# chto/linna

Measured on AMD Instinct MI355X. Metric: emulator log-likelihood evals/sec, higher is better.
Workload: dtype f32; 1 GPU; 33-D Gaussian, 4x512 MLP emulator (33->512x4->33), nwalkers=4096 batched log-likelihood per GPU (BASELINE configs[1]); nwalkers_per_gpu=4096, launch=direct launches, parallelism=walkers sharded, 1 rank(s), no data-path collective

## Files before the change

### linna_amd/csrc/net_stream.hip

```cpp
#include "common.h"
#include <stdlib.h>
#include <type_traits>
#include <vector>
#include <cstring>
#include <algorithm>
#include <atomic>
#include <memory>
#include <mutex>
#include <string>
#include <unordered_map>

namespace linna {

typedef __bf16 bf16x8 __attribute__((ext_vector_type(8)));
typedef short s16x4 __attribute__((ext_vector_type(4)));

constexpr int NS_ROWS = 16;
constexpr int NS_NW = 8;
constexpr int NS_NT = 4;
constexpr int NS_MAXSEG = 20;
constexpr int NS_MAXRUN = 40;
constexpr unsigned NS_STEP_B = NS_NT * 1024;
constexpr int NS_LDS_BYTES = 160 * 1024;
#ifndef NS_R
// ... 412 lines not shown
            in_ext[i] = (NS_NW / ncg) * s.kslice;
            q.bias_pad = 64 * ncg; q.ncg = ncg;
        } else {
            s.type = NS_WIDE; s.steps = ksteps; s.passes = passes;
            in_ext[i] = KS * ksteps;
            q.bias_pad = 512 * passes; q.ncg = 1;
        }
        q.Wa = L.Wa; q.lda = L.lda; q.Ka = L.Ka; q.Kapad = L.Kapad; q.Wb = L.Wb; q.ldb = L.ldb; q.Kb = L.Kb; q.alpha = L.alpha;
        q.b = L.b; q.bscale = L.bscale; q.N = L.N; q.type = s.type; q.steps = s.steps; q.passes = s.passes; q.bias_off = bias_off;
        q.transA = L.transA; q.transB = L.transB; q.rscale = L.rscale; q.rshift = L.rshift; q.b2 = L.b2; q.b2scale = L.b2scale;
        q.kc = side ? kc : 1; q.side_off = 0;
        s.x0_col = L.x0_col; s.x0_n = L.x0_col ? ceil16(L.Kb) : 0;
        if (L.transA && !dx_prog) {
            if (zero_off < 0) { zero_off = bias_off; zero_pad = 0; }
            s.bias_off = q.bias_off = zero_off;
            const int grow = std::max(0, q.bias_pad - zero_pad);
            zero_pad += grow; q.bias_pad = grow;
        }
        bias_off += q.bias_pad;
        if (dn && dn->tri > 0 && s.type == NS_WIDE && dn->factored && L.Wa == dn->S && passes == 2 && ksteps > 32 && !train) {
            if (dn->tri == 2 && (L.N + 63) / 64 == 16 && ksteps > 60) s.zext = -1;
            else { s.kslice = 512; s.zext = ksteps - 32; }
        }
        q.koff2 = s.type == NS_WIDE ? (s.zext < 0 ? -1 : s.kslice) : 0;
        if (!side) G += ns_seg_steps(s);
        p.seg.push_back(s); p.pack.push_back(q);
    }
    if (want_grad) {
        int slot = 0;
        for (int i = 0; i < nfwd - 1; ++i) {
            if (p.seg[i].type != NS_WIDE) { want_grad = false; break; }
            p.seg[i].mask_store = 1 + slot;
            slot += p.seg[i].passes;
        }
        for (size_t j = nfwd; j < lins.size() && want_grad; ++j) {
            const int of = lins[j].mask_apply_of;
            if (of < 0) continue;
            if (p.seg[j].type != NS_WIDE || p.seg[j].passes != p.seg[of].passes) { want_grad = false; break; }
            p.seg[j].mask_apply = p.seg[of].mask_store;
        }
        if (want_grad) p.mask_slots = slot;
        else {
            for (size_t j = lins.size(); j-- > (size_t)nfwd;) { G -= ns_seg_steps(p.seg[j]); bias_off -= p.pack[j].bias_pad; }
            p.seg.resize(nfwd); p.pack.resize(nfwd); lins.resize(nfwd); in_ext.resize(nfwd);
            for (int i = 0; i < nfwd; ++i) p.seg[i].mask_store = 0;
        }
    }
    int Gf = 0;
    for (int i = 0; i < nfwd; ++i) if (p.seg[i].type != NS_SIDE) Gf += ns_seg_steps(p.seg[i]);

    p.kpad0 = in_ext[0];
    int def = p.kpad0, writer = -1;
    int maxext = 64;
    for (size_t i = 0; i < p.seg.size(); ++i) {
        NsSeg& s = p.seg[i];
        if (in_ext[i] > def) {
            if (writer == -1) p.kpad0 = def = in_ext[i];
            else if (writer >= 0) { NsSeg& w = p.seg[writer]; w.zext = in_ext[i] - w.dst_col; def = in_ext[i]; }
            else return p;
        }
        maxext = std::max(maxext, in_ext[i]);
        if (s.type == NS_WIDE) {
            if (s.dst_col != 0) return p;
            def = 512 * s.passes; writer = -2;
            maxext = std::max(maxext, def);
        } else {
            if (s.dst_col > def) return p;
            if (s.dst_col == 0) def = s.zext;
            else def = std::max(def, s.dst_col + s.zext);
            writer = (int)i;
        }
    }
    for (const NsSeg& s : p.seg) if (s.type != NS_WIDE) maxext = std::max(maxext, s.dst_col + s.zext);
    if (p.kpad0 > (dx_prog ? 1024 : bf ? 512 : 256)) return p;
    p.bf = bf; p.f32seg = f32seg;
    p.nout = lins[nfwd - 1].N;
    p.G = Gf; p.Gstride = G; p.nseg_f = nfwd; p.grad_ok = want_grad;
    for (size_t i = 0; i < lins.size(); ++i) { p.seg_op.push_back(lins[i].op); p.seg_hidden.push_back(lins[i].same_buf ? 1 : 0); }
    p.dxi_ok = fwd_dxi;
    p.train_ok = train;
    p.bias_total = bias_off;
    p.LD = std::max(((maxext + 63) & ~63) + 4, 516);
    if (bias_off > 3 * 64 * NS_NW * 4) return p;
    p.lds_bytes = (size_t)(2 * NS_ROWS * p.LD + ((bias_off + 3) & ~3)) * sizeof(float) + 128 + (p.x0_keep ? 4096 : 0);
#ifdef NS_STAMPS
    p.lds_bytes += NS_NW * 32 * 8;
#endif
    if (p.lds_bytes > (size_t)NS_LDS_BYTES) return p;
    p.lds_bytes_grad = p.lds_bytes + (size_t)p.mask_slots * 64 * NS_NW * sizeof(unsigned);
    if (p.grad_ok && p.lds_bytes_grad > (size_t)NS_LDS_BYTES) return p;
    int nrun = 0;
    for (const NsSeg& s : p.seg) nrun += s.passes;
    if (nrun > NS_MAXRUN) return p;
    p.packed_floats = (size_t)NS_NW * G * NS_NT * 256 + (size_t)((bias_off + 3) & ~3);
    for (size_t i = 0; i < p.seg.size(); ++i)
        if (p.seg[i].type == NS_SIDE) {
            p.seg[i].side_off = p.pack[i].side_off = (int)p.packed_floats;
            p.packed_floats += (size_t)NS_NW * p.seg[i].steps * NS_NT * 256;
            p.side_f4 += (size_t)NS_NW * p.seg[i].steps * NS_NT * 64;
        }
    p.ok = true;
    return p;
}

static std::atomic<int> g_forced_rows{-1};
static int ns_forced_rows_resolved() {
    int forced = g_forced_rows.load(std::memory_order_relaxed);
    if (forced < 0) {
        const char* const env = getenv("LINNA_NS_ROWS");
        const int v = env ? atoi(env) : 0;
        forced = (v == 4 || v == 8 || v == 16) ? v : 0;
        int expect = -1;
        g_forced_rows.compare_exchange_strong(expect, forced);
        forced = g_forced_rows.load(std::memory_order_relaxed);
    }
    return forced;
}
int net_stream_force_rows(int rows) {
    if (rows != 0 && rows != 4 && rows != 8 && rows != 16) return -1;
    (void)ns_forced_rows_resolved();
    return g_forced_rows.exchange(rows);
}
int net_stream_rows(int B) {
    const int forced = ns_forced_rows_resolved();
    if (forced) return forced;
    static int ncu = 0;
    if (!ncu) {
        int dev = 0; hipDeviceProp_t pr;
        ncu = (hipGetDevice(&dev) == hipSuccess && hipGetDeviceProperties(&pr, dev) == hipSuccess && pr.multiProcessorCount > 0)
                  ? pr.multiProcessorCount : 256;
    }
    return B <= 4 * ncu ? 4 : B <= 8 * ncu ? 8 : 16;
}

static bool ns_side(NsKind kind, int rows) {
    return rows == 16 && (kind == NS_SERVE || kind == NS_SERVE_DENSE || kind == NS_GRAD_INPUT);
}

static NsProgram ns_build_kind(NsKind kind, const linna_layer_t* layers, int nl, int in_size, const NsDense* dn, bool side) {
    NsProgram p;
    switch (kind) {
    case NS_SERVE: case NS_STORE:
        p = ns_build_one(layers, nl, in_size, NS_PROG_FWD, nullptr, side);
        if (!p.ok) p = ns_build_one(layers, nl, in_size, NS_PROG_FWD_NOGRAD, nullptr, side);
        break;
    case NS_SERVE_DENSE: case NS_TRAIN_FWD: p = ns_build_one(layers, nl, in_size, NS_PROG_FWD_DENSE, dn, side); break;
    case NS_SERVE_BF16: p = ns_build_one(layers, nl, in_size, NS_PROG_FWD_NOGRAD, dn, false, true); break;
    case NS_DX: p = ns_build_one(layers, nl, in_size, NS_PROG_DX); break;
    case NS_DX_INPUT: p = ns_build_one(layers, nl, in_size, NS_PROG_DX_INPUT); break;
    case NS_GRAD_INPUT: p = ns_build_one(layers, nl, in_size, NS_PROG_FWD_DXI, nullptr, side); break;
    case NS_TRAIN_STEP: p = ns_build_one(layers, nl, in_size, NS_PROG_TRAIN, dn); break;
    case NS_TRAIN_STEP_BF16: p = ns_build_one(layers, nl, in_size, NS_PROG_TRAIN, dn, false, true); break;
    }
    if (side && !(p.ok && (kind != NS_GRAD_INPUT || p.dxi_ok))) return ns_build_kind(kind, layers, nl, in_size, dn, false);
    return p;
}
typedef std::shared_ptr<const NsProgram> NsProgramRef;
static NsProgramRef ns_program(NsKind kind, const linna_layer_t* layers, int nl, int in_size, const NsDense* dn, int rows) {
    static std::mutex mu;
    static std::unordered_map<std::string, NsProgramRef> cache;
    const bool side = ns_side(kind, rows);
    std::string key;
    key.reserve((size_t)nl * sizeof(linna_layer_t) + 64);
    key.append(reinterpret_cast<const char*>(layers), (size_t)nl * sizeof(linna_layer_t));
    const int hdr[4] = {nl, in_size, (int)kind, side ? 1 : 0};
    key.append(reinterpret_cast<const char*>(hdr), sizeof(hdr));
// ... 586 lines not shown
```

### linna_amd/csrc/net_stream_body.inc

```
    constexpr int NT = NS_NT, NW = NS_NW;
    constexpr int RG = 32;
    constexpr bool SM = ROWS < 16;
    constexpr int RS = SM ? ROWS / 4 : 1;
    constexpr int NQ = SM ? RS : NT;
    constexpr int NACC = SM ? 4 * RS : NT;
#ifdef NS_BODY_SLICE_BF16
    static_assert(BF && !GRAD && STORE == 0 && MOVE == 2, "bf16: the slice evaluation");
#else
    static_assert(!BF || (!GRAD && STORE == 0 && MOVE != 2) || (GRAD && STORE == 3 && MOVE == 0 && ROWS == 4),
                  "bf16: serving, the fused stretch move and the merged training step (4-row engine)");
#endif
    constexpr bool BFT = BF && GRAD && STORE == 3;
    constexpr int AK = BF ? 2 : 1;
    constexpr bool K4 = !SM && !BF && (STORE == 0 || (GRAD && STORE == 2));
    constexpr bool TRB = GRAD && STORE == 3;
    constexpr bool DXE = STORE == 2 || TRB;
    constexpr bool G2 = GRAD && STORE == 2;
    constexpr bool LB = G2;
    constexpr bool LATE_REFILL = true;
    static_assert(ROWS == 16 || ROWS == 8 || ROWS == 4, "rows per workgroup");
    static_assert(R % 2 == 0, "the A double buffer alternates with the ring slot parity");
    extern __shared__ __attribute__((aligned(16))) float smem[];
    const int LD = a.LD, ABUF = ROWS * LD;
    constexpr bool KA = STORE == 3 || STORE == 1 || GRAD;
    const NsArgs* const ka = KA ? reinterpret_cast<const NsArgs*>((const void*)__builtin_amdgcn_kernarg_segment_ptr()) : &a;
    float* const act = smem;
    float* const lbias = smem + 2 * ABUF;
    unsigned* const lbits = reinterpret_cast<unsigned*>(smem + a.bits_off);
    const int nbw = a.nbw;
    const int tid = threadIdx.x, lane = tid & 63;
    const int wave = __builtin_amdgcn_readfirstlane(tid >> 6);
    const int li = lane & 15, kq = lane >> 4;
    const int row0 = blockIdx.x * ROWS;
    if (a.gate && a.gate[0] == 0) return;
    int mv_rows = a.B;
    if constexpr (MOVE == 2) {
        if (a.mv_C) {
            mv_rows = a.mv_step[0] * a.mv_step_off;
            if (row0 >= mv_rows) return;
        }
    }
    if constexpr ((STORE == 2 && !GRAD) || TRB) {
        if ((a.p_n > 0 || a.p_step) && blockIdx.x == gridDim.x - 1) {
            float* const part = smem;
            float acc0 = 0.f, acc1 = 0.f;
            for (int i = tid; i < a.p_n; i += 1024) acc0 += a.p_rows[i];
            for (int i = tid + 512; i < a.p_n; i += 1024) acc1 += a.p_rows[i];
#pragma unroll
            for (int o = 32; o >= 1; o >>= 1) { acc0 += __shfl_xor(acc0, o, 64); acc1 += __shfl_xor(acc1, o, 64); }
            if (lane == 0) { part[wave] = acc0; part[8 + wave] = acc1; }
            __syncthreads();
            if (tid == 0 && a.p_out) {
                float t = 0.f;
                for (int w = 0; w < 16; ++w) t += part[w];
                a.p_out[0] = t * a.p_scale;
            }
            if (tid == 64 && a.p_step) {
                const int t = ++a.p_step[0];
                a.p_hyper[2] = (float)(1.0 - pow((double)a.p_b1, (double)t));
                a.p_hyper[3] = (float)sqrt(1.0 - pow((double)a.p_b2, (double)t));
            }
            return;
        }
    }
#ifdef NS_STAMPS
    unsigned long long* const lstamp = reinterpret_cast<unsigned long long*>(lbias + ((a.bias_total + 3) & ~3) + 32 + (a.x0_keep ? 1024 : 0)) + wave * 32;
    int nstamp = 0;
#define NS_STAMP() do { const unsigned long long t_ = __builtin_readcyclecounter(); \
        if (lane == 0 && nstamp < 32) lstamp[nstamp] = t_; ++nstamp; } while (0)
#define NS_STAMPS_FLUSH() do { if (lane < 32) a.stamps[((size_t)blockIdx.x * NW + wave) * 32 + lane] = lane < nstamp ? lstamp[lane] : 0ull; } while (0)
#else
#define NS_STAMP() do {} while (0)
#define NS_STAMPS_FLUSH() do {} while (0)
#endif
    NS_STAMP();

    const int prt = tid / RG, pc0 = tid % RG;
    const bool prow = prt < ROWS;
    const int pr = SM ? min(prt, ROWS - 1) : prt;
    int grow = min(row0 + pr, a.B - 1);
    if constexpr (MOVE == 2) {
        if (a.mv_C) grow = a.mv_C[min(row0 + pr, mv_rows - 1)];
    }
    int zsrc = grow;
    float zden = 1.f;
    if constexpr (STORE == 3) {
        zsrc = a.t_rows ? a.t_rows[grow] : grow;
        zden = a.t_den[zsrc];
    }
    const int kpad0 = a.kpad0, nin = a.nin, nout = a.nout, nseg = a.nseg;
    const int nlast = (TRB ? a.nseg_f : nseg) - 2;
    constexpr int ZPRE = 2;
    float zr[ZPRE], za1[ZPRE], za2[ZPRE], zxm[ZPRE], zxs[ZPRE]; int zfl[ZPRE], zlg[ZPRE];
    const int* const lgp = a.lg ? a.lg : a.is_flat;
    int mv_wk = 0; float mv_factor = 0.f, mv_lnp_old = 0.f, mv_logu = 0.f;
    if constexpr (MOVE == 1) {
        mv_wk = a.mv_S[grow];
        const U4 rb = walker_bits(a.mv_seed, (uint32_t)mv_wk, (uint32_t)(a.mv_step[0] + a.mv_step_off), (uint32_t)a.mv_stream, 0u);
        const float t = (a.mv_a - 1.f) * u01(rb.x) + 1.f;
        const float zf = t * t / a.mv_a;
        const int j = (int)(((uint64_t)rb.y * (uint64_t)a.mv_nc) >> 32);
        const int wc = a.mv_C[j];
// ... 3 lines not shown
#pragma unroll
        for (int i = 0; i < ZPRE; ++i) {
            const int c = min(pc0 + i * RG, nin - 1);
            const float cr = a.mv_cc[(size_t)wc * a.mv_ldcc + c], sx = a.mv_coords[(size_t)mv_wk * a.mv_ldc + c];
            zr[i] = cr - (cr - sx) * zf;
        }
    }
    if constexpr (MOVE == 2) {
        const int k = grow % a.mv_nc;
        const int wk = a.mv_S[k];
        float wgt;
        if (a.sb.logp) {
            const SliceBegin& b = a.sb;
            const int jt = grow / a.mv_nc;
            const U4 rb = walker_bits(b.seed, (uint32_t)wk, (uint32_t)b.step[0], (uint32_t)b.half, 0u);
            const int ia = (int)(((uint64_t)rb.x * (uint64_t)b.nc) >> 32);
            int ib = (int)(((uint64_t)rb.y * (uint64_t)(b.nc - 1)) >> 32);
            ib += (ib >= ia);
            const int wa = b.C[ia], wb = b.C[ib];
            const float mu = b.mu[0];
            const float l = -u01(rb.w);
            wgt = jt < b.m ? l - (float)jt : l + 1.f + (float)(jt - b.m);
            const bool first = jt == 0 && prow && row0 + pr < a.B;
#pragma unroll
            for (int i = 0; i < ZPRE; ++i) {
                const int c = min(pc0 + i * RG, nin - 1);
                const float dir = mu * (b.cc[(size_t)wa * b.ldcc + c] - b.cc[(size_t)wb * b.ldcc + c]);
                zr[i] = a.mv_coords[(size_t)wk * a.mv_ldc + c] + wgt * dir;
                if (first && pc0 + i * RG < nin) b.DIR[(size_t)k * b.ldd + c] = dir;
            }
            if (first && pc0 == 0) {
                b.Z0[k] = b.logp[wk] + logf(u01(rb.z));
                b.L[k] = l; b.R[k] = l + 1.f;
                int J, K;
                slice_budget(b.seed, (uint32_t)wk, (uint32_t)b.step[0], (uint32_t)b.half, b.maxsteps, J, K);
                b.flags[3 * k] = J; b.flags[3 * k + 1] = K; b.flags[3 * k + 2] = 1;
            }
            if (blockIdx.x == 0 && tid == 0) {
                for (int i = 0; i < b.nslots; ++i) {
                    b.counters[4 + b.nslots + i] += b.counters[4 + i];
                    b.counters[4 + i] = 0;
                }
                b.counters[4 + 2 * b.nslots] += 1;
                if (b.zero_totals) { b.counters[0] = 0; b.counters[1] = 0; }
            }
        } else {
        if (a.sl_Zt) {
            const int ns_ = a.mv_nc, m = a.sl_m, jt = grow / ns_;
            const float z0 = a.sl_Z0[k];
            const float zend = a.sl_Zt[(size_t)min(pc0, 2 * m - 1) * ns_ + k];
            const unsigned long long bal = __ballot(pc0 < 2 * m && zend > z0);
            const unsigned bits = (unsigned)(bal >> (lane & 32));
            const unsigned lm = bits & ((1u << m) - 1u), rm = (bits >> m) & ((1u << m) - 1u);
            const int nl = min(__builtin_ctz(~lm), a.sl_flags[3 * k]), nr = min(__builtin_ctz(~rm), a.sl_flags[3 * k + 1]);
            float l = a.sl_L[k], r = a.sl_R[k];
            for (int j = 0; j < m; ++j) {
                if (j < nl) l -= 1.f;
                if (j < nr) r += 1.f;
            }
            const U4 tb = walker_bits(a.sl_seed, (uint32_t)wk, (uint32_t)a.sl_step[0], (uint32_t)a.sl_stream, (uint32_t)(pc0 + 1));
            const int myu = __float_as_int(u01(tb.x));
            wgt = 0.f;
            for (int jj = 0; jj < a.sl_nt; ++jj) {
                const int ulo = __builtin_amdgcn_readlane(myu, jj), uhi = __builtin_amdgcn_readlane(myu, 32 + jj);
                const float u = __int_as_float((lane & 32) ? uhi : ulo);
                const float w = l + u * (r - l);
                if (jj == jt) wgt = w;
                if (jj < jt) { if (w < 0.f) l = w; else r = w; }
            }
        } else {
            wgt = a.mv_cc[grow];
        }
#pragma unroll
        for (int i = 0; i < ZPRE; ++i) {
            const int c = min(pc0 + i * RG, nin - 1);
            zr[i] = a.mv_coords[(size_t)wk * a.mv_ldc + c] + wgt * a.Z[(size_t)k * a.ldz + c];
        }
        }
    }
#pragma unroll
    for (int i = 0; i < ZPRE; ++i) {
        const int c = min(pc0 + i * RG, nin - 1);
        if constexpr (MOVE == 0) zr[i] = a.Z[(size_t)(STORE == 3 ? zsrc : grow) * a.ldz + c];
        zfl[i] = a.is_flat[c]; za1[i] = a.a1[c]; za2[i] = a.a2[c];
        zlg[i] = lgp[c]; zxm[i] = a.xmean[c]; zxs[i] = a.xstd[c];
    }
    const int nb4 = (a.bias_total + 3) >> 2;
    const f32x4* const bsrc = reinterpret_cast<const f32x4*>(a.packed + (size_t)NW * a.Gstride * NT * 256);
    constexpr int BMAX = 3;
    f32x4 breg[BMAX];
#pragma unroll
    for (int i = 0; i < BMAX; ++i) {
        const int j = tid + i * 64 * NW;
        breg[i] = bsrc[min(j, nb4 - 1)];
    }
    constexpr int FIN = 2;
    const float* const csp = a.cscale ? a.cscale : a.xmean;
    const float* const ctp = a.cshift ? a.cshift : a.xmean;
    const float* const wtp = a.w ? a.w : a.xmean;
    float fcs[FIN], fct[FIN], fw[FIN], fgs[FIN];
#pragma unroll
    for (int i = 0; i < FIN; ++i) {
        const int cc = min(pc0 + i * RG, nout - 1);
        if constexpr (GRAD && !TRB) fgs[i] = a.gscale[cc]; else fgs[i] = 0.f;
        const int c1 = a.cscale ? cc : 0, c2 = a.cshift ? cc : 0, c3 = a.w ? cc : 0;
        const float cs = csp[c1], ct = ctp[c2], ww = wtp[c3];
        fcs[i] = a.cscale ? cs : 1.f; fct[i] = a.cshift ? ct : 0.f; fw[i] = a.w ? ww : 0.f;
    }

    const char* const wbase = reinterpret_cast<const char*>(a.packed) + (size_t)wave * a.Gstride * NS_STEP_B;
    const unsigned wlast = (unsigned)(a.G - 1) * NS_STEP_B;
    unsigned woff = 0;
    const unsigned voff = 16u * (unsigned)lane;
    f32x4 Bq[R][NT];
    auto wload = [&](int t) { return *reinterpret_cast<const f32x4*>(wbase + (size_t)(voff + woff) + t * 1024); };
    auto wadvance = [&]() { woff = min(woff + NS_STEP_B, wlast); };
    constexpr int PRE = NS_PRE < R ? NS_PRE : R;
    auto prefetch = [&](auto Uc) {
        constexpr int U = decltype(Uc)::value;
#pragma unroll
        for (int t = 0; t < NT; ++t) {
            Bq[U][t] = wload(t);
            __builtin_amdgcn_sched_barrier(0);
        }
        wadvance();
    };
#define NS_PF(U, LO, HI) if constexpr (U >= LO && U < HI) prefetch(std::integral_constant<int, U>{});
#define NS_PF_ALL(LO, HI) NS_PF(0, LO, HI) NS_PF(1, LO, HI) NS_PF(2, LO, HI) NS_PF(3, LO, HI) NS_PF(4, LO, HI) NS_PF(5, LO, HI) \
    NS_PF(6, LO, HI) NS_PF(7, LO, HI)
    NS_PF_ALL(0, PRE)
#ifdef NS_STAMPS_FINE
    NS_STAMP();
#endif

    float zz = 0.f;
    float theta[ZPRE];
#pragma unroll
    for (int i = 0; i < ZPRE; ++i) {
        const int c = pc0 + i * RG;
        const bool in = c < nin;
        const float z = in ? zr[i] : 0.f;
        zz += z * z;
        float th = ns_prior_theta(z, zfl[i], za1[i], za2[i]);
        float lt = log10f(th);
        asm volatile("" : "+v"(lt));
        theta[i] = th;
        const float t = (a.lg && zlg[i]) ? lt : th;
        float x = in ? (t - zxm[i]) / zxs[i] : 0.f;
        if constexpr ((STORE == 1 || STORE == 2) && !GRAD) x = z;
        if constexpr (STORE == 3) {
            float lz = log10f(z);
            asm volatile("" : "+v"(lz));
            const float tz = (a.lg && zlg[i]) ? lz : z;
            x = in ? (tz - zxm[i]) / zxs[i] : 0.f;
            if (prow && row0 + pr < a.B && c < a.t_ldxb)
                asm volatile("global_store_dword %0, %1, off" :: "v"(a.t_xb + (size_t)(row0 + pr) * a.t_ldxb + c), "v"(x) : "memory");
        }
        if constexpr (BF) {
            if (prow) {
                if (in) { const float hi = (float)(__bf16)x; act[pr * LD + c] = hi; act[pr * LD + nin + c] = x - hi; }
                else if (c >= 2 * nin && c < kpad0) act[pr * LD + c] = 0.f;
            }
        } else {
            if (c < kpad0 && prow) act[pr * LD + c] = x;
        }
    }
#ifdef NS_STAMPS_FINE
    NS_STAMP();
#endif
    if constexpr ((STORE == 1 || STORE == 2) && !GRAD) {
        const int wcols = kpad0 - ZPRE * RG;
        if (wcols > 0) {
            constexpr int CP = 4;
            for (int base = 0; base < ROWS * wcols; base += CP * 64 * NW) {
                float v[CP];
#pragma unroll
                for (int u = 0; u < CP; ++u) {
                    const int idx = min(base + u * 64 * NW + tid, ROWS * wcols - 1);
                    const int r = idx / wcols, c = ZPRE * RG + idx % wcols;
                    v[u] = a.Z[(size_t)min(row0 + r, a.B - 1) * a.ldz + min(c, nin - 1)];
                }
#pragma unroll
                for (int u = 0; u < CP; ++u) {
                    const int idx = base + u * 64 * NW + tid;
                    if (idx < ROWS * wcols) {
                        const int r = idx / wcols, c = ZPRE * RG + idx % wcols;
                        act[r * LD + c] = c < nin ? v[u] : 0.f;
                    }
                }
            }
        }
    } else
#pragma unroll 1
    for (int c = pc0 + ZPRE * RG; c < kpad0; c += RG) {
        float x = 0.f;
        if (c < nin) {
            const float z = a.Z[(size_t)grow * a.ldz + c];
            zz += z * z;
            const float th = ns_prior_theta(z, a.is_flat[c], a.a1[c], a.a2[c]);
            const float t = (a.lg && a.lg[c]) ? log10f(th) : th;
            x = (t - a.xmean[c]) / a.xstd[c];
            if constexpr ((STORE == 1 || STORE == 2) && !GRAD) x = z;
            if constexpr (STORE == 3) {
                const float zz3 = a.Z[(size_t)zsrc * a.ldz + c];
                x = (((a.lg && a.lg[c]) ? log10f(zz3) : zz3) - a.xmean[c]) / a.xstd[c];
            }
        }
        if constexpr (STORE == 3) {
            if (prow && row0 + pr < a.B && c < a.t_ldxb)
                asm volatile("global_store_dword %0, %1, off" :: "v"(a.t_xb + (size_t)(row0 + pr) * a.t_ldxb + c), "v"(x) : "memory");
        }
        if constexpr (BF) {
            if (prow) {
                if (c < nin) { const float hi = (float)(__bf16)x; act[pr * LD + c] = hi; act[pr * LD + nin + c] = x - hi; }
                else if (c >= 2 * nin) act[pr * LD + c] = 0.f;
            }
        } else {
            if (prow) act[pr * LD + c] = x;
        }
    }
    __builtin_amdgcn_sched_barrier(0);
#ifdef NS_STAMPS_FINE
    NS_STAMP();
#endif
    NS_PF_ALL(PRE, (LATE_REFILL ? R - 1 : R))
#undef NS_PF_ALL
#undef NS_PF
#pragma unroll
    for (int o = RG / 2; o >= 1; o >>= 1) zz += __shfl_xor(zz, o, 64);
#pragma unroll
    for (int i = 0; i < BMAX; ++i) {
        const int j = tid + i * 64 * NW;
        if (j < nb4) reinterpret_cast<f32x4*>(lbias)[j] = breg[i];
    }
    int* const lsrc = reinterpret_cast<int*>(lbias + ((a.bias_total + 3) & ~3));
    float* const lden = reinterpret_cast<float*>(lsrc + 16);
    if constexpr (STORE == 3) {
        if (prow && pc0 == 0) { lsrc[pr] = zsrc; lden[pr] = zden; }
    }
    float* const lx0 = lden + 16;
    if (a.x0_keep && prow) {
#pragma unroll
        for (int i = 0; i < ZPRE; ++i) {
            const int c = pc0 + i * RG;
            if constexpr (BF) lx0[pr * 64 + c] = c < nin ? act[pr * LD + c] + act[pr * LD + nin + c] : 0.f;
            else lx0[pr * 64 + c] = (c < kpad0) ? act[pr * LD + c] : 0.f;
        }
    }
    asm volatile("s_waitcnt lgkmcnt(0)" ::: "memory");
    __builtin_amdgcn_s_barrier();
    asm volatile("" ::: "memory");
    NS_STAMP();

    const uint32_t act_lds = (uint32_t)(uintptr_t)(__attribute__((address_space(3))) void*)act;
    f32x4 acc[NACC];
    f32x4 Aq[2][AK];
    const int sm_arow = (4 * ((lane >> 2) & 3) + (lane & 3)) % ROWS, sm_achunk = lane >> 4;
    int si = 0, pass = 0, P = 0, kleft;
    int s_type, s_steps, s_passes, s_bias, s_dst, s_relu, s_kslice, s_zext, s_ncgl, s_mstore = 0, s_mapply = 0, s_x0col = 0, s_x0n = 0, s_kcl = 0;
    unsigned* const lmask = reinterpret_cast<unsigned*>(lbias + ((a.bias_total + 3) & ~3));
    float lnp_grad = 0.f;
    float* s_gout = nullptr; int s_gld = 0, s_gn = 0;
    const float* s_gmask = nullptr; int s_gmld = 0;
    int s_gbit = -1, s_mbit = -1;
    auto gstore = [&](float* p, float v) { asm volatile("global_store_dword %0, %1, off" :: "v"(p), "v"(v) : "memory"); };
    uint32_t ap;
    auto a_read = [&](f32x4* dst) {
        asm volatile("ds_read_b128 %0, %1" : "=v"(dst[0]) : "v"(ap) : "memory");
        if constexpr (BF) asm volatile("ds_read_b128 %0, %1 offset:16" : "=v"(dst[1]) : "v"(ap) : "memory");
        if constexpr (BFT) ap += si == a.nseg_f - 1 ? 64 : 64 * AK;
        else ap += 64 * AK;
    };
    auto load_seg = [&]() {
        const NsSeg S = ka->seg[__builtin_amdgcn_readfirstlane(si)];
        s_type = S.type; kleft = s_steps = S.steps; s_passes = S.passes; s_bias = S.bias_off;
        s_dst = S.dst_col; s_relu = S.relu; s_kslice = S.kslice; s_zext = S.zext; s_ncgl = S.ncg_log2; s_x0col = S.x0_col; s_x0n = S.x0_n;
        if constexpr (GRAD) { s_mstore = S.mask_store; s_mapply = S.mask_apply; }
        if constexpr (STORE) { const int j = __builtin_amdgcn_readfirstlane(si); s_gout = ka->gout[j]; s_gld = ka->gld[j]; s_gn = ka->gn[j]; }
        if constexpr (DXE) { const int j = __builtin_amdgcn_readfirstlane(si); s_gmask = ka->gmask[j]; s_gmld = ka->gmld[j]; }
        if constexpr (LB) { const int j = __builtin_amdgcn_readfirstlane(si); s_gbit = ka->gbit[j]; s_mbit = ka->mbit[j]; }
    };
    auto begin_run = [&]() {
        const int arow = SM ? sm_arow : li, ak = AK * (SM ? 4 * sm_achunk : 4 * kq);
#pragma unroll
        for (int t = 0; t < NACC; ++t) acc[t] = f32x4{0.f, 0.f, 0.f, 0.f};
        if (s_type == NS_WIDE) {
            const int blk = s_zext < 0 ? (pass ? 15 - wave : wave) : 8 * pass + wave;
            if constexpr (SM) {
                const float b = lbias[s_bias + 64 * blk + lane];
#pragma unroll
                for (int r = 0; r < RS; ++r) acc[4 * r] = f32x4{b, b, b, b};
            } else {
#pragma unroll
                for (int t = 0; t < NT; ++t) {
                    const float b = lbias[s_bias + 16 * (4 * blk + t) + li];
                    acc[t] = f32x4{b, b, b, b};
                }
            }
            if (s_zext < 0) kleft = s_steps - 4 * blk;
            ap = act_lds + 4u * (uint32_t)(P * ABUF + arow * LD + ak + (s_zext < 0 ? 64 * blk : (pass ? s_kslice : 0)));
        } else {
            ap = act_lds + 4u * (uint32_t)(P * ABUF + arow * LD + ak + (wave >> s_ncgl) * s_kslice);
        }
        if constexpr (BFT) {
            if (si == a.nseg_f - 1) ap -= 4u * (uint32_t)(ak / 2);
        }
    };
    auto lds_barrier = [&]() {
        asm volatile("s_waitcnt lgkmcnt(0)" ::: "memory");
        __builtin_amdgcn_s_barrier();
        asm volatile("" ::: "memory");
    };
    load_seg();
    begin_run();
    a_read(Aq[0]);

    auto step = [&](auto Uc, auto Refill) {
        constexpr int U = decltype(Uc)::value;
        constexpr bool refill = decltype(Refill)::value;
        constexpr int RU = LATE_REFILL ? (U + R - 1) % R : U;
        if constexpr (BF) asm volatile("s_waitcnt lgkmcnt(0)" : "+v"(Aq[U & 1][0]), "+v"(Aq[U & 1][AK - 1]) :: "memory");
        else asm volatile("s_waitcnt lgkmcnt(0)" : "+v"(Aq[U & 1][0]) :: "memory");
        a_read(Aq[(U + 1) & 1]);
        const f32x4 av = Aq[U & 1][0];
        if constexpr (BF) {
            bf16x8 ab;
#pragma unroll
            for (int e = 0; e < 4; ++e) { ab[e] = (__bf16)Aq[U & 1][0][e]; ab[4 + e] = (__bf16)Aq[U & 1][AK - 1][e]; }
            if constexpr (SM) {
                auto bf_small = [&]() {
                    const s16x4 alo = __builtin_bit_cast(s16x4, __builtin_shufflevector(ab, ab, 0, 1, 2, 3));
                    const s16x4 ahi = __builtin_bit_cast(s16x4, __builtin_shufflevector(ab, ab, 4, 5, 6, 7));
#define NS_B4(r, c, h, A4) acc[4 * (r) + (c)] = __builtin_amdgcn_mfma_f32_4x4x4bf16_1k(A4, \
                __builtin_bit_cast(s16x4, __builtin_shufflevector(__builtin_bit_cast(bf16x8, Bq[U][c]), __builtin_bit_cast(bf16x8, Bq[U][c]), \
                                                                  4 * (h), 4 * (h) + 1, 4 * (h) + 2, 4 * (h) + 3)), acc[4 * (r) + (c)], 4, 4 * (c) + (r), 0);
#define NS_B4R(r, h, A4) NS_B4(r, 0, h, A4) NS_B4(r, 1, h, A4) NS_B4(r, 2, h, A4) NS_B4(r, 3, h, A4)
                    NS_B4R(0, 0, alo)
                    if constexpr (RS > 1) { NS_B4R(1, 0, alo) }
                    NS_B4R(0, 1, ahi)
                    if constexpr (RS > 1) { NS_B4R(1, 1, ahi) }
#undef NS_B4R
#undef NS_B4
                };
                if constexpr (BFT) {
                    if (si == a.nseg_f - 1) {
#define NS_M4(r, c, e) acc[4 * (r) + (c)] = __builtin_amdgcn_mfma_f32_4x4x1f32(av[e], Bq[U][c][e], acc[4 * (r) + (c)], 4, 4 * (c) + (r), 0);
#define NS_M4R(r, e) NS_M4(r, 0, e) NS_M4(r, 1, e) NS_M4(r, 2, e) NS_M4(r, 3, e)
#pragma unroll
                        for (int e = 0; e < 4; ++e) {
                            NS_M4R(0, e)
                            if constexpr (RS > 1) { NS_M4R(1, e) }
                        }
#undef NS_M4R
#undef NS_M4
                    } else {
                        bf_small();
                    }
                } else {
                    bf_small();
                }
                if constexpr (refill) {
#pragma unroll
                    for (int t = 0; t < NT; ++t) Bq[RU][t] = wload(t);
                }
            } else {
#pragma unroll
                for (int h = 0; h < NT; h += 2) {
                    acc[h] = __builtin_amdgcn_mfma_f32_16x16x32_bf16(ab, __builtin_bit_cast(bf16x8, Bq[U][h]), acc[h], 0, 0, 0);
                    acc[h + 1] = __builtin_amdgcn_mfma_f32_16x16x32_bf16(ab, __builtin_bit_cast(bf16x8, Bq[U][h + 1]), acc[h + 1], 0, 0, 0);
                    if constexpr (refill) {
                        Bq[RU][h] = wload(h);
                        Bq[RU][h + 1] = wload(h + 1);
                    }
                }
            }
        } else if constexpr (SM) {
#define NS_M4(r, c, e) acc[4 * (r) + (c)] = __builtin_amdgcn_mfma_f32_4x4x1f32(av[e], Bq[U][c][e], acc[4 * (r) + (c)], 4, 4 * (c) + (r), 0);
#define NS_M4R(r, e) NS_M4(r, 0, e) NS_M4(r, 1, e) NS_M4(r, 2, e) NS_M4(r, 3, e)
#pragma unroll
            for (int e = 0; e < 4; ++e) {
                NS_M4R(0, e)
                if constexpr (RS > 1) { NS_M4R(1, e) }
            }
#undef NS_M4R
#undef NS_M4
            if constexpr (refill) {
#pragma unroll
                for (int t = 0; t < NT; ++t) Bq[RU][t] = wload(t);
            }
        } else {
#pragma unroll
            for (int h = 0; h < NT; h += 2) {
#pragma unroll
                for (int s = 0; s < 4; ++s) {
                    acc[h] = __builtin_amdgcn_mfma_f32_16x16x4f32(av[s], Bq[U][h][s], acc[h], 0, 0, 0);
                    acc[h + 1] = __builtin_amdgcn_mfma_f32_16x16x4f32(av[s], Bq[U][h + 1][s], acc[h + 1], 0, 0, 0);
                }
                if constexpr (refill) {
                    Bq[RU][h] = wload(h);
                    Bq[RU][h + 1] = wload(h + 1);
                }
            }
        }
        if constexpr (refill) wadvance();
        if (--kleft == 0) {
            const int nxi = __builtin_amdgcn_readfirstlane(min(si + 1, nseg - 1));
            const NsSeg NX = ka->seg[nxi];
            float* nx_gout = nullptr; int nx_gld = 0, nx_gn = 0;
            const float* nx_gmask = nullptr; int nx_gmld = 0;
            if constexpr (STORE) { nx_gout = ka->gout[nxi]; nx_gld = ka->gld[nxi]; nx_gn = ka->gn[nxi]; }
            if constexpr (DXE) { nx_gmask = ka->gmask[nxi]; nx_gmld = ka->gmld[nxi]; }
            int nx_gbit = -1, nx_mbit = -1;
            if constexpr (LB) { nx_gbit = ka->gbit[nxi]; nx_mbit = ka->mbit[nxi]; }
            const int cur_steps = s_steps;
            auto take_seg = [&](const NsSeg& X) {
                s_type = X.type; s_steps = X.steps; s_passes = X.passes; s_bias = X.bias_off;
                s_dst = X.dst_col; s_relu = X.relu; s_kslice = X.kslice; s_zext = X.zext; s_ncgl = X.ncg_log2; s_x0col = X.x0_col; s_x0n = X.x0_n;
                if constexpr (K4) s_kcl = X.kcl;
                if constexpr (GRAD) { s_mstore = X.mask_store; s_mapply = X.mask_apply; }
                kleft = X.steps;
            };
            auto take_next = [&]() {
                take_seg(NX);
                if constexpr (STORE) { s_gout = nx_gout; s_gld = nx_gld; s_gn = nx_gn; }
                if constexpr (DXE) { s_gmask = nx_gmask; s_gmld = nx_gmld; }
                if constexpr (LB) { s_gbit = nx_gbit; s_mbit = nx_mbit; }
            };
            f32x4 sdw[2][NT];
            bool side_next = false;
            if constexpr (K4) {
#pragma unroll
                for (int s2 = 0; s2 < 2; ++s2)
#pragma unroll
                    for (int t = 0; t < NT; ++t) sdw[s2][t] = f32x4{0.f, 0.f, 0.f, 0.f};
                if (NX.type == NS_SIDE && si + 1 < nseg && (s_type != NS_WIDE || pass + 1 == s_passes)) {
                    side_next = true;
                    const char* const sb = reinterpret_cast<const char*>(a.packed + NX.side_off) + (size_t)wave * NX.steps * NS_STEP_B + voff;
#pragma unroll
                    for (int t = 0; t < NT; ++t)
                        asm volatile("global_load_dwordx4 %0, %1, off" : "=v"(sdw[0][t]) : "v"(sb + t * 1024) : "memory");
                    if (NX.steps > 1) {
#pragma unroll
                        for (int t = 0; t < NT; ++t)
                            asm volatile("global_load_dwordx4 %0, %1, off" : "=v"(sdw[1][t]) : "v"(sb + NS_STEP_B + t * 1024) : "memory");
                    }
                }
            }
            bool seg_done = true;
#ifdef NS_STAMPS_FINE
            const bool fine = si >= NS_STAMPS_FINE && si < NS_STAMPS_FINE + 4;
            if (fine) NS_STAMP();
#endif
            if constexpr (SM) {
#pragma unroll
                for (int q = 0; q < NQ; ++q) acc[q] = (acc[4 * q] + acc[4 * q + 1]) + (acc[4 * q + 2] + acc[4 * q + 3]);
            }
#define fin acc
#define q_row(q, e) (SM ? 4 * (q) + (e) : 4 * kq + (e))
#define q_col(q) (SM ? lane : 16 * (q) + li)
            if (s_type == NS_WIDE) {
                float* const nxt = act + (P ^ 1) * ABUF + s_dst + (s_zext < 0 ? 64 * (pass ? 15 - wave : wave) : 512 * pass + 64 * wave);
                float ty[NQ][4];
                if constexpr (STORE == 3) {
                    if (si == nlast) {
#pragma unroll
                        for (int t = 0; t < NQ; ++t) {
                            const int dc = min(512 * pass + 64 * wave + q_col(t), nout - 1);
#pragma unroll
                            for (int e = 0; e < 4; ++e) {
                                const float* py = a.t_Y + (size_t)lsrc[q_row(t, e)] * a.t_ldy + dc;
                                asm volatile("global_load_dword %0, %1, off" : "=v"(ty[t][e]) : "v"(py) : "memory");
                            }
                        }
#pragma unroll
                        for (int t = 0; t < NQ; ++t)
                            asm volatile("s_waitcnt vmcnt(0)" : "+v"(ty[t][0]), "+v"(ty[t][1]), "+v"(ty[t][2]), "+v"(ty[t][3]) :: "memory");
                    }
                }
                unsigned long long gw[SM ? NQ : 1][4];
                if constexpr (LB) {
                    if (s_mbit >= 0) {
                        const int cw = 512 * pass + 64 * wave, w0 = (s_mbit + cw) >> 5;
                        const bool mine = cw < ((s_gn + 63) & ~63);
#pragma unroll
                        for (int t = 0; t < (SM ? NQ : 1); ++t)
#pragma unroll
                            for (int e = 0; e < 4; ++e)
                                gw[t][e] = mine ? *reinterpret_cast<const unsigned long long*>(lbits + (SM ? 4 * t + e : 4 * kq + e) * nbw + w0) : 0ull;
                    }
                }
                if constexpr (DXE && !LB) {
                    if (s_gmask) {
#pragma unroll
                        for (int t = 0; t < NQ; ++t) {
                            const int mc = min(512 * pass + 64 * wave + q_col(t), s_gn - 1);
#pragma unroll
                            for (int e = 0; e < 4; ++e) {
                                const float* pg = s_gmask + (size_t)min(row0 + q_row(t, e), a.B - 1) * s_gmld + mc;
                                if constexpr (GRAD)
                                    asm volatile("global_load_dword %0, %1, off sc1" : "=v"(ty[t][e]) : "v"(pg) : "memory");
                                else
                                    asm volatile("global_load_dword %0, %1, off" : "=v"(ty[t][e]) : "v"(pg) : "memory");
                            }
                        }
#pragma unroll
                        for (int t = 0; t < NQ; ++t)
                            asm volatile("s_waitcnt vmcnt(0)" : "+v"(ty[t][0]), "+v"(ty[t][1]), "+v"(ty[t][2]), "+v"(ty[t][3]) :: "memory");
                    }
                }
                unsigned mbits = 0xFFFFu;
                if constexpr (GRAD) {
                    if (s_mapply) mbits = lmask[(s_mapply - 1 + pass) * (64 * NW) + threadIdx.x];
                    if (s_mstore) {
                        unsigned m = 0;
#pragma unroll
                        for (int t = 0; t < NQ; ++t)
#pragma unroll
                            for (int e = 0; e < 4; ++e) m |= (fin[t][e] > 0.f ? 1u : 0u) << (4 * t + e);
                        lmask[(s_mstore - 1 + pass) * (64 * NW) + threadIdx.x] = m;
                    }
                }
#pragma unroll
                for (int t = 0; t < NQ; ++t)
#pragma unroll
                    for (int e = 0; e < 4; ++e) {
                        float v = fin[t][e];
                        if constexpr (GRAD) v = ((mbits >> (4 * t + e)) & 1u) ? v : 0.f;
                        v = s_relu ? fmaxf(v, 0.f) : v;
                        if constexpr (LB) {
                            if (s_mbit >= 0 && !((gw[SM ? t : 0][e] >> (SM ? lane : 16 * t + li)) & 1ull)) v = 0.f;
                        } else if constexpr (DXE) {
                            if (s_gmask && !(ty[t][e] > 0.f)) v = 0.f;
                        }
                        float v_lds = v;
                        if constexpr (STORE == 3) {
                            if (si == nlast) {
                                const int dc = 512 * pass + 64 * wave + q_col(t);
                                const float yn = ty[t][e];
                                v_lds = dc < nout ? (isnan(yn) ? -0.f : (yn - v) + 0.f) : 0.f;
                            }
                        }
                        nxt[q_row(t, e) * LD + q_col(t)] = v_lds;
                        if constexpr (LB) {
                            if (s_gbit >= 0) {
                                const unsigned long long bb = __ballot(v > 0.f);
                                const int cw = 512 * pass + 64 * wave;
                                const bool mine = cw < ((s_gn + 63) & ~63);
                                const int c0 = s_gbit + cw;
                                if constexpr (SM) {
                                    if (lane == 0 && mine) *reinterpret_cast<unsigned long long*>(lbits + (4 * t + e) * nbw + (c0 >> 5)) = bb;
                                } else {
                                    if (li == 0 && mine) reinterpret_cast<unsigned short*>(lbits + (4 * kq + e) * nbw)[(c0 + 16 * t) >> 4] = (unsigned short)(bb >> (16 * kq));
                                }
                            }
                        }
                        if constexpr (STORE && !G2) {
                            const int grow_ = row0 + q_row(t, e), gcol = 512 * pass + 64 * wave + q_col(t);
                            if (s_gout && grow_ < a.B && gcol < s_gn) {
                                float vs = v;
                                if constexpr (STORE == 1)
                                    if (si == nseg - 1) vs = vs * (a.cscale ? a.cscale[gcol] : 1.f) + (a.cshift ? a.cshift[gcol] : 0.f);
                                gstore(s_gout + (size_t)grow_ * s_gld + gcol, vs);
                            }
                        }
                    }
#ifdef NS_STAMPS_FINE
                if (fine) NS_STAMP();
#endif
                if (++pass == s_passes) {
                    lds_barrier();
                    NS_STAMP();
                    P ^= 1; pass = 0; ++si;
                    take_next();
                } else {
                    kleft = s_zext > 0 ? s_zext : cur_steps;
                    seg_done = false;
                }
            } else {
                float* const part = act + (P ^ 1) * ABUF;
                constexpr int PW = ROWS * 64;
#pragma unroll
                for (int t = 0; t < NQ; ++t)
#pragma unroll
                    for (int e = 0; e < 4; ++e) {
                        const int rr = q_row(t, e);
                        part[wave * PW + rr * 64 + (q_col(t) ^ (SM ? 32 * (rr & 1) : 16 * kq))] = fin[t][e];
                    }
#ifdef NS_STAMPS_FINE
                if (fine) NS_STAMP();
#endif
                lds_barrier();
#ifdef NS_STAMPS_FINE
                if (fine) NS_STAMP();
#endif
                constexpr int RGS = SM ? 64 * NW / ROWS : RG;
                const int sr = SM ? tid / RGS : pr, sc0 = SM ? tid % RGS : pc0;
                const bool srow = SM ? true : prow;
                float* const cur = act + P * ABUF + sr * LD + s_dst;
                const int ncol = 64 << s_ncgl, nkp = NW >> s_ncgl;
                const int sw = SM ? 32 * (sr & 1) : 16 * (sr >> 2);
                constexpr int NGJ = 256 / RGS;
                float sg[NGJ];
                if constexpr (DXE && !LB) {
                    if (s_gmask) {
#pragma unroll
                        for (int j = 0; j < NGJ; ++j) {
                            const float* pg = s_gmask + (size_t)min(row0 + sr, a.B - 1) * s_gmld + min(sc0 + RGS * j, s_gn - 1);
                            if constexpr (GRAD)
                                asm volatile("global_load_dword %0, %1, off sc1" : "=v"(sg[j]) : "v"(pg) : "memory");
                            else
                                asm volatile("global_load_dword %0, %1, off" : "=v"(sg[j]) : "v"(pg) : "memory");
                        }
#pragma unroll
                        for (int j = 0; j < NGJ; ++j) asm volatile("s_waitcnt vmcnt(0)" : "+v"(sg[j]) :: "memory");
                    }
                }
                int gj = 0;
                if constexpr ((!LB && !DXE && !STORE) || (LB && !SM)) {
                    auto reduce4 = [&](auto NKc) {
                        constexpr int NK = decltype(NKc)::value;
                        for (int c = 4 * sc0; c < (srow ? s_zext : 0); c += 4 * RGS) {
                            f32x4 v = f32x4{0.f, 0.f, 0.f, 0.f};
                            if (c < ncol) {
                                const float* src = part + (c >> 6) * PW + sr * 64 + ((c & 63) ^ sw);
                                constexpr int CH = LB && NK > 4 ? 4 : NK;
                                const f32x4 b = *reinterpret_cast<const f32x4*>(lbias + s_bias + c);
#pragma unroll
                                for (int k0 = 0; k0 < NK; k0 += CH) {
                                    f32x4 x[CH];
#pragma unroll
                                    for (int kp = 0; kp < CH; ++kp) x[kp] = *reinterpret_cast<const f32x4*>(src + ((k0 + kp) << s_ncgl) * PW);
#pragma unroll
                                    for (int kp = 0; kp < CH; ++kp) v += x[kp];
                                }
                                v += b;
                                if (s_relu) v = f32x4{fmaxf(v[0], 0.f), fmaxf(v[1], 0.f), fmaxf(v[2], 0.f), fmaxf(v[3], 0.f)};
                            }
                            if constexpr (LB) {
                                const bool mine = c < ((s_gn + 63) & ~63);
                                if (s_mbit >= 0) {
                                    const unsigned nib = mine ? (lbits[sr * nbw + ((s_mbit + c) >> 5)] >> (c & 31)) & 0xFu : 0u;
#pragma unroll
                                    for (int e = 0; e < 4; ++e) v[e] = ((nib >> e) & 1u) ? v[e] : 0.f;
                                }
                                *reinterpret_cast<f32x4*>(cur + c) = v;
                                if (s_gbit >= 0) {
                                    unsigned w32 = ((v[0] > 0.f ? 1u : 0u) | (v[1] > 0.f ? 2u : 0u) | (v[2] > 0.f ? 4u : 0u) | (v[3] > 0.f ? 8u : 0u)) << (c & 31);
                                    w32 |= __shfl_xor(w32, 1, 64); w32 |= __shfl_xor(w32, 2, 64); w32 |= __shfl_xor(w32, 4, 64);
                                    if ((sc0 & 7) == 0 && mine) lbits[sr * nbw + ((s_gbit + c) >> 5)] = w32;
                                }
                            } else {
                                *reinterpret_cast<f32x4*>(cur + c) = v;
                            }
                        }
                    };
                    if (nkp == NW) reduce4(std::integral_constant<int, NW>{});
                    else if (nkp == NW / 2) reduce4(std::integral_constant<int, NW / 2>{});
                    else reduce4(std::integral_constant<int, 2>{});
                } else
                for (int c = sc0; c < (srow ? s_zext : 0); c += RGS, ++gj) {
                    float v = 0.f;
                    if (c < ncol) {
                        const float* src = part + (c >> 6) * PW + sr * 64 + ((c & 63) ^ sw);
// ... 272 lines not shown
        const float* const Dv = a.u_same ? F : act + (P ^ 1) * ABUF + pr * LD;
        const float* const Uv = a.u_same ? F + a.u_col : F;
        float chi = 0.f;
        for (int c = pc0; c < nout; c += RG) chi += Dv[c] * Uv[c];
#pragma unroll
        for (int o = RG / 2; o >= 1; o >>= 1) chi += __shfl_xor(chi, o, 64);
        if (rok && pc0 == 0) a.t_loss_rows[row0 + pr] = chi / lden[pr];
        {
            constexpr int TPR = 64 * NW / ROWS;
            const int fr = tid / TPR, fc = tid % TPR;
            if (row0 + fr < a.B) {
                const float* const Fr = act + P * ABUF + fr * LD;
                const float* const Dr = a.u_same ? Fr : act + (P ^ 1) * ABUF + fr * LD;
                const float* const Ur = a.u_same ? Fr + a.u_col : Fr;
                const float dr = lden[fr];
                for (int c = fc; c < a.t_lddp; c += TPR) {
                    float g = 0.f;
                    if (c < nout) {
                        const bool masked = __float_as_uint(Dr[c]) == 0x80000000u;
                        g = masked ? 0.f : (-2.f * Ur[c]) * a.t_inv_batch / dr;
                    }
                    a.t_dP[(size_t)(row0 + fr) * a.t_lddp + c] = g;
                }
            }
        }
        NS_STAMP();
        NS_STAMPS_FLUSH();
        return;
    }
    if constexpr (GRAD) {
        const float* const F = act + P * ABUF + pr * LD;
        const bool rok = prow && row0 + pr < a.B;
        if (rok) {
#pragma unroll
            for (int j = 0; j < ZPRE; ++j) {
                const int c = pc0 + j * RG;
                if (c < nin) {
                    float g = F[c] / zxs[j];
                    if (a.lg && zlg[j]) g = g / (theta[j] * 2.30258509299404568f);
                    const float z = zr[j];
                    const float dth = zfl[j] ? za2[j] * (expf(-0.5f * z * z) * 0.398942280401432678f) : za2[j];
                    const float gz = g * dth - z;
                    a.Gout[(size_t)(row0 + pr) * a.ldg + c] = gz;
                    if (a.hm_p) {
                        float* const pp = a.hm_p + (size_t)(row0 + pr) * a.hm_ldp + c;
                        float pm = *pp;
                        if (a.hm_ek != 0.f) { pm += a.hm_ek * gz; *pp = pm; }
                        if (a.hm_ed != 0.f) a.hm_q[(size_t)(row0 + pr) * a.ldz + c] = z + a.hm_ed * (pm / a.hm_mass[c]);
                    }
                }
            }
            if (pc0 == 0) a.lnP[row0 + pr] = isnan(lnp_grad) ? -INFINITY : lnp_grad;
        }
        if constexpr (STORE == 2) { NS_STAMP(); NS_STAMPS_FLUSH(); }
        return;
    }
    {
        const float* const F = act + P * ABUF + pr * LD;
        const bool rok = prow && row0 + pr < a.B;
        float chi = 0.f;
        auto column = [&](int c, float cs, float ct, float ww) {
            float d = F[c] * cs + ct;
            if (a.cpost) d = expf(d) * a.cpost[c] + a.cshift2[c];
            if (a.D && rok) a.D[(size_t)(row0 + pr) * a.ldd + c] = d;
            chi += (d * ww) * d;
        };
        if (a.dense) {
            const float* const Dv = a.u_same ? F : act + (P ^ 1) * ABUF + pr * LD;
            const float* const U = a.u_same ? F + a.u_col : F;
            const bool fac = a.dense == 2;
            for (int c = pc0; c < nout; c += RG) {
                const float d = Dv[c];
                if (a.D && rok) a.D[(size_t)(row0 + pr) * a.ldd + c] = d;
                const float u = U[c];
                chi += (fac ? u : d) * u;
            }
        } else {
#pragma unroll
            for (int i = 0; i < FIN; ++i)
                if (pc0 + i * RG < nout) column(pc0 + i * RG, fcs[i], fct[i], fw[i]);
            for (int c = pc0 + FIN * RG; c < nout; c += RG)
                column(c, a.cscale ? a.cscale[c] : 1.f, a.cshift ? a.cshift[c] : 0.f, a.w ? a.w[c] : 0.f);
        }
#pragma unroll
        for (int o = RG / 2; o >= 1; o >>= 1) chi += __shfl_xor(chi, o, 64);
        float lnp_new = (-0.5f * chi) / a.T + (-0.5f * zz);
        lnp_new = isnan(lnp_new) ? -INFINITY : lnp_new;
        if constexpr (MOVE == 2) {
            if (a.lnP && pc0 == 0 && prow && row0 + pr < mv_rows) a.lnP[a.mv_C ? grow : row0 + pr] = lnp_new;
        } else {
            if (a.lnP && (a.w || a.dense) && pc0 == 0 && rok) a.lnP[row0 + pr] = lnp_new;
        }
        if constexpr (MOVE == 1) {
            const bool mv_acc = rok && mv_factor + lnp_new - mv_lnp_old > mv_logu;
            if (mv_acc) {
#pragma unroll
                for (int j = 0; j < ZPRE; ++j)
                    if (pc0 + j * RG < nin) a.mv_coords[(size_t)mv_wk * a.mv_ldc + pc0 + j * RG] = zr[j];
                if (pc0 == 0) {
                    a.mv_logp[mv_wk] = lnp_new;
                    if (a.mv_naccept) a.mv_naccept[mv_wk] += 1;
                }
            }
            if (a.mv_chain && rok) {
#pragma unroll
                for (int j = 0; j < ZPRE; ++j)
                    if (pc0 + j * RG < nin)
                        a.mv_chain[(size_t)mv_wk * nin + pc0 + j * RG] = mv_acc ? zr[j] : a.mv_coords[(size_t)mv_wk * a.mv_ldc + pc0 + j * RG];
                if (pc0 == 0) a.mv_lps[mv_wk] = mv_acc ? lnp_new : mv_lnp_old;
            }
        }
        if (a.TH && rok) {
#pragma unroll
            for (int j = 0; j < ZPRE; ++j)
                if (pc0 + j * RG < nin) a.TH[(size_t)(row0 + pr) * a.ldt + pc0 + j * RG] = theta[j];
            for (int c = pc0 + ZPRE * RG; c < nin; c += RG)
                a.TH[(size_t)(row0 + pr) * a.ldt + c] = ns_prior_theta(a.Z[(size_t)grow * a.ldz + c], a.is_flat[c], a.a1[c], a.a2[c]);
        }
    }
    NS_STAMP();
    NS_STAMPS_FLUSH();
#undef NS_STAMP
#undef NS_STAMPS_FLUSH
```

Baseline: 72.85 million evals/s.

## Transpose MFMA operands for vectorized LDS stores and cooperative header loads

For the 16-row f32 serving path, MFMA operand order is swapped so each lane holds four consecutive columns. This lets bias init, activation writeback and partial sums use f32x4 LDS accesses instead of scalar ones. Per-column prior/normalization parameters are now loaded once per workgroup, each wave fetching one array and sharing it through LDS, rather than every lane doing many scalar global loads. The change also skips log10f when the log flag is off, uses DPP for the 32-lane reductions, adjusts the prefetch depth, and adds alignment guards on LD and segment offsets.

```diff
diff --git a/linna_amd/csrc/net_stream.hip b/linna_amd/csrc/net_stream.hip
--- a/linna_amd/csrc/net_stream.hip
+++ b/linna_amd/csrc/net_stream.hip
@@ -518,6 +518,8 @@
     p.bias_total = bias_off;
     p.LD = std::max(((maxext + 63) & ~63) + 4, 516);
     if (bias_off > 3 * 64 * NS_NW * 4) return p;
+    if (p.LD % 4) return p;
+    for (const NsSeg& s : p.seg) if (s.dst_col % 4 || s.bias_off % 4) return p;
     p.lds_bytes = (size_t)(2 * NS_ROWS * p.LD + ((bias_off + 3) & ~3)) * sizeof(float) + 128 + (p.x0_keep ? 4096 : 0);
 #ifdef NS_STAMPS
     p.lds_bytes += NS_NW * 32 * 8;
diff --git a/linna_amd/csrc/net_stream_body.inc b/linna_amd/csrc/net_stream_body.inc
--- a/linna_amd/csrc/net_stream_body.inc
+++ b/linna_amd/csrc/net_stream_body.inc
@@ -18,6 +18,19 @@
     constexpr bool G2 = GRAD && STORE == 2;
     constexpr bool LB = G2;
     constexpr bool LATE_REFILL = true;
+    constexpr bool TA = !GRAD && STORE == 0 && !BF && ROWS == 16;
+    constexpr bool HC = TA, LS = TA, DR = TA;
+    auto reduce32_dpp = [](float v) {
+        auto dpp_add = [](float x, auto ctrl) {
+            return x + __int_as_float(__builtin_amdgcn_update_dpp(0, __float_as_int(x), decltype(ctrl)::value, 0xF, 0xF, false));
+        };
+        v += __shfl_xor(v, 16, 64);
+        v = dpp_add(v, std::integral_constant<int, 0x128>{});
+        v = dpp_add(v, std::integral_constant<int, 0x124>{});
+        v = dpp_add(v, std::integral_constant<int, 0x4E>{});
+        v = dpp_add(v, std::integral_constant<int, 0xB1>{});
+        return v;
+    };
     static_assert(ROWS == 16 || ROWS == 8 || ROWS == 4, "rows per workgroup");
     static_assert(R % 2 == 0, "the A double buffer alternates with the ring slot parity");
     extern __shared__ __attribute__((aligned(16))) float smem[];
@@ -187,8 +200,21 @@
     for (int i = 0; i < ZPRE; ++i) {
         const int c = min(pc0 + i * RG, nin - 1);
         if constexpr (MOVE == 0) zr[i] = a.Z[(size_t)(STORE == 3 ? zsrc : grow) * a.ldz + c];
-        zfl[i] = a.is_flat[c]; za1[i] = a.a1[c]; za2[i] = a.a2[c];
-        zlg[i] = lgp[c]; zxm[i] = a.xmean[c]; zxs[i] = a.xstd[c];
+        if constexpr (!HC) {
+            zfl[i] = a.is_flat[c]; za1[i] = a.a1[c]; za2[i] = a.a2[c];
+            zlg[i] = lgp[c]; zxm[i] = a.xmean[c]; zxs[i] = a.xstd[c];
+        }
+    }
+    unsigned hc0 = 0, hc1 = 0;
+    if constexpr (HC) {
+        const int ci = min(lane, nin - 1), co = min(lane, nout - 1);
+        const void* const hp = wave == 0 ? (const void*)(a.is_flat + ci) : wave == 1 ? (const void*)(a.a1 + ci)
+                             : wave == 2 ? (const void*)(a.a2 + ci)      : wave == 3 ? (const void*)(lgp + ci)
+                             : wave == 4 ? (const void*)(a.xmean + ci)   : wave == 5 ? (const void*)(a.xstd + ci)
+                             : wave == 6 ? (const void*)(a.cscale ? a.cscale + co : a.xmean)
+                                         : (const void*)(a.cshift ? a.cshift + co : a.xmean);
+        hc0 = *reinterpret_cast<const unsigned*>(hp);
+        hc1 = *reinterpret_cast<const unsigned*>(a.w ? a.w + co : a.xmean);
     }
     const int nb4 = (a.bias_total + 3) >> 2;
     const f32x4* const bsrc = reinterpret_cast<const f32x4*>(a.packed + (size_t)NW * a.Gstride * NT * 256);
@@ -204,6 +230,7 @@
     const float* const ctp = a.cshift ? a.cshift : a.xmean;
     const float* const wtp = a.w ? a.w : a.xmean;
     float fcs[FIN], fct[FIN], fw[FIN], fgs[FIN];
+    if constexpr (!HC)
 #pragma unroll
     for (int i = 0; i < FIN; ++i) {
         const int cc = min(pc0 + i * RG, nout - 1);
@@ -220,7 +247,7 @@
     f32x4 Bq[R][NT];
     auto wload = [&](int t) { return *reinterpret_cast<const f32x4*>(wbase + (size_t)(voff + woff) + t * 1024); };
     auto wadvance = [&]() { woff = min(woff + NS_STEP_B, wlast); };
-    constexpr int PRE = NS_PRE < R ? NS_PRE : R;
+    constexpr int PRE = HC ? (LATE_REFILL ? R - 1 : R) : NS_PRE < R ? NS_PRE : R;
     auto prefetch = [&](auto Uc) {
         constexpr int U = decltype(Uc)::value;
 #pragma unroll
@@ -237,6 +264,24 @@
 #ifdef NS_STAMPS_FINE
     NS_STAMP();
 #endif
+    if constexpr (HC) {
+        unsigned* const hcb = reinterpret_cast<unsigned*>(act + ABUF);
+        if (wave < 6) hcb[8 * lane + wave] = hc0;
+        else hcb[512 + 4 * lane + (wave - 6)] = wave == 6 ? (a.cscale ? hc0 : __float_as_uint(1.f)) : (a.cshift ? hc0 : 0u);
+        if (wave == 0) hcb[512 + 4 * lane + 2] = a.w ? hc1 : 0u;
+        asm volatile("s_waitcnt lgkmcnt(0)" ::: "memory");
+        __builtin_amdgcn_s_barrier();
+        asm volatile("" ::: "memory");
+#pragma unroll
+        for (int i = 0; i < ZPRE; ++i) {
+            const int c = pc0 + i * RG;
+            const f32x4 p0 = *reinterpret_cast<const f32x4*>(hcb + 8 * c), p1 = *reinterpret_cast<const f32x4*>(hcb + 8 * c + 4);
+            const f32x4 po = *reinterpret_cast<const f32x4*>(hcb + 512 + 4 * c);
+            zfl[i] = __float_as_int(p0[0]); za1[i] = p0[1]; za2[i] = p0[2]; zlg[i] = __float_as_int(p0[3]);
+            zxm[i] = p1[0]; zxs[i] = p1[1];
+            fcs[i] = po[0]; fct[i] = po[1]; fw[i] = po[2]; fgs[i] = 0.f;
+        }
+    }
 
     float zz = 0.f;
     float theta[ZPRE];
@@ -247,8 +292,11 @@
         const float z = in ? zr[i] : 0.f;
         zz += z * z;
         float th = ns_prior_theta(z, zfl[i], za1[i], za2[i]);
-        float lt = log10f(th);
-        asm volatile("" : "+v"(lt));
+        float lt = th;
+        if (!LS || a.lg) {
+            lt = log10f(th);
+            asm volatile("" : "+v"(lt));
+        }
         theta[i] = th;
         const float t = (a.lg && zlg[i]) ? lt : th;
         float x = in ? (t - zxm[i]) / zxs[i] : 0.f;
@@ -331,6 +379,8 @@
     NS_PF_ALL(PRE, (LATE_REFILL ? R - 1 : R))
 #undef NS_PF_ALL
 #undef NS_PF
+    if constexpr (DR) zz = reduce32_dpp(zz);
+    else
 #pragma unroll
     for (int o = RG / 2; o >= 1; o >>= 1) zz += __shfl_xor(zz, o, 64);
 #pragma unroll
@@ -398,8 +448,12 @@
             } else {
 #pragma unroll
                 for (int t = 0; t < NT; ++t) {
-                    const float b = lbias[s_bias + 16 * (4 * blk + t) + li];
-                    acc[t] = f32x4{b, b, b, b};
+                    if constexpr (TA) {
+                        acc[t] = *reinterpret_cast<const f32x4*>(lbias + s_bias + 16 * (4 * blk + t) + 4 * kq);
+                    } else {
+                        const float b = lbias[s_bias + 16 * (4 * blk + t) + li];
+                        acc[t] = f32x4{b, b, b, b};
+                    }
                 }
             }
             if (s_zext < 0) kleft = s_steps - 4 * blk;
@@ -498,8 +552,13 @@
             for (int h = 0; h < NT; h += 2) {
 #pragma unroll
                 for (int s = 0; s < 4; ++s) {
-                    acc[h] = __builtin_amdgcn_mfma_f32_16x16x4f32(av[s], Bq[U][h][s], acc[h], 0, 0, 0);
-                    acc[h + 1] = __builtin_amdgcn_mfma_f32_16x16x4f32(av[s], Bq[U][h + 1][s], acc[h + 1], 0, 0, 0);
+                    if constexpr (TA) {
+                        acc[h] = __builtin_amdgcn_mfma_f32_16x16x4f32(Bq[U][h][s], av[s], acc[h], 0, 0, 0);
+                        acc[h + 1] = __builtin_amdgcn_mfma_f32_16x16x4f32(Bq[U][h + 1][s], av[s], acc[h + 1], 0, 0, 0);
+                    } else {
+                        acc[h] = __builtin_amdgcn_mfma_f32_16x16x4f32(av[s], Bq[U][h][s], acc[h], 0, 0, 0);
+                        acc[h + 1] = __builtin_amdgcn_mfma_f32_16x16x4f32(av[s], Bq[U][h + 1][s], acc[h + 1], 0, 0, 0);
+                    }
                 }
                 if constexpr (refill) {
                     Bq[RU][h] = wload(h);
@@ -625,6 +684,18 @@
                         lmask[(s_mstore - 1 + pass) * (64 * NW) + threadIdx.x] = m;
                     }
                 }
+                if constexpr (TA) {
+                    float* const wp = nxt + li * LD + 4 * kq;
+#pragma unroll
+                    for (int t = 0; t < NT; ++t) {
+                        f32x4 v = fin[t];
+                        if (s_relu) {
+#pragma unroll
+                            for (int e = 0; e < 4; ++e) asm("v_max_f32 %0, 0, %1" : "=v"(v[e]) : "v"(fin[t][e]));
+                        }
+                        *reinterpret_cast<f32x4*>(wp + 16 * t) = v;
+                    }
+                } else
 #pragma unroll
                 for (int t = 0; t < NQ; ++t)
 #pragma unroll
@@ -684,6 +755,11 @@
             } else {
                 float* const part = act + (P ^ 1) * ABUF;
                 constexpr int PW = ROWS * 64;
+                if constexpr (TA) {
+#pragma unroll
+                    for (int t = 0; t < NT; ++t)
+                        *reinterpret_cast<f32x4*>(part + wave * PW + li * 64 + ((16 * t + 4 * kq) ^ (16 * (li >> 2)))) = fin[t];
+                } else
 #pragma unroll
                 for (int t = 0; t < NQ; ++t)
 #pragma unroll
@@ -1122,6 +1198,8 @@
             for (int c = pc0 + FIN * RG; c < nout; c += RG)
                 column(c, a.cscale ? a.cscale[c] : 1.f, a.cshift ? a.cshift[c] : 0.f, a.w ? a.w[c] : 0.f);
         }
+        if constexpr (DR) chi = reduce32_dpp(chi);
+        else
 #pragma unroll
         for (int o = RG / 2; o >= 1; o >>= 1) chi += __shfl_xor(chi, o, 64);
         float lnp_new = (-0.5f * chi) / a.T + (-0.5f * zz);
```

Result: no change. 72.52 million evals/s (-0.5%).
